# main--/rust-lz-fear

Hardware: AMD Instinct MI355X
Metric: GiB/s compress + decompress, 4 MiB independent blocks, 1/2/4/8 MI355X (higher is better)
Workload: dtype u8

## Files before the change

rust-lz-fear_amd/build.py:

```python
import hashlib
import os
import subprocess
from concurrent.futures import ThreadPoolExecutor

PKG_DIR = os.path.dirname(os.path.abspath(__file__))
CSRC = os.path.join(PKG_DIR, "csrc")
ROOT = os.path.dirname(PKG_DIR)
LIB_PATH = os.environ.get("LZF_LIB_PATH") or os.path.join(PKG_DIR, "liblzfear_hip.so")
ANALYSIS_LIB_PATH = os.path.join(PKG_DIR, "liblzfear_hip_analysis.so")

PRODUCT_HIP = ["capi.hip", "lz4_decompress_batched.hip", "lz4_decompress_paired.hip", "lz4_decompress_seg.hip", "lz4_decompress_fed.hip", "lz4_decoded_size.hip", "lz4_compress.hip",
               "lz4_compress_compact.hip", "lz4_compress_team.hip", "aux_kernels.hip", "frame_device.hip"]
ANALYSIS_HIP = ["analysis/lz4_decompress.hip"]
CXX_SOURCES = ["frame.cpp", "host_staging.cpp"]
HEADERS = ["kernels.h", "lzf_device.h", "lz4_decompress_batch_phase.inc", "lz4_decompress_parse_phase.inc", "lz4_decompress_feed_phase.inc",
           "analysis/capi_analysis.inc",
           "lzf_copy_helpers.h", "lzf_parse_helpers.h", "lzf_compress_common.h", "lzf_simt.h", "lz4_compress_team.inc",
           "host_staging.h", "lzf_frame_scan.h", "lzf_stream_walk.h", "frame_jobs.h", "lzf_frame_layout.h", "lzf_size_rules.h", "lzf_chain_step.h", "frame_deliver_body.inc",
           os.path.join(ROOT, "include", "lzfear_hip.h"), os.path.join(ROOT, "include", "lzfear_frame.h")]


def _path(d):
    return d if os.path.isabs(d) else os.path.join(CSRC, d)


def hipcc():
    for c in ("/opt/rocm/bin/hipcc", "hipcc"):
        if os.path.isabs(c) and os.path.exists(c):
            return c
    return "hipcc"


def _sources(analysis):
# ... 89 lines not shown
```

rust-lz-fear_amd/csrc/capi.hip:

```cpp
#include <hip/hip_runtime.h>
#include <cstdio>
#include <cstdlib>
#include <cstring>
#include <string>
#include <mutex>
#include <vector>
#include "kernels.h"
#include "host_staging.h"

namespace {

thread_local std::string g_last_error;
thread_local const char* g_last_decompress = "";
thread_local const char* g_last_compress = "";

int fail_hip(hipError_t e, const char* what) {
    char buf[256];
    snprintf(buf, sizeof buf, "%s: %s", what, hipGetErrorString(e));
    g_last_error = buf;
    return LZF_E_HIP;
}
#define HIP_TRY(expr)                                          \
    do {                                                       \
        hipError_t e__ = (expr);                               \
// ... 346 lines not shown
    (void)hipGetLastError();
    if (!answer.slots) {
        const uint32_t by_lds = per_cu(kFedLdsAlloc);
        answer.slots = (by_lds < kFedWavesPerCu ? by_lds : kFedWavesPerCu) * cu_count();
    }
#ifdef LZF_ANALYSIS
    if (getenv("LZF_FED_VERBOSE")) fprintf(stderr, "[lzf] bitmap-fed kernel: %u workgroups resident at once (%u compute units), XCD mask 0x%x\n", answer.slots, cu_count(), answer.xcc_mask);
#endif
    by_dev[dev] = answer;
    return answer;
}
struct FedCall {
    SegScratch s; const lzf_decompress_job* jobs = nullptr; lzf_job_result* res = nullptr; uint32_t n = 0; const uint32_t* perm = nullptr;
    size_t o_tick = 0, o_fst = 0; bool live = false;
};
int fed_front(FedCall& f, const lzf_decompress_job* d_jobs, lzf_job_result* d_results, uint32_t n, const uint32_t* perm, hipStream_t st, uint64_t max_in_hint) {
    f.jobs = d_jobs; f.res = d_results; f.n = n; f.perm = perm; f.live = false;
    lzf::seg_ctx& c = f.s.ctx;
    c = lzf::seg_ctx{};
    c.jobs = d_jobs; c.results = d_results; c.n_jobs = n;
    const uint32_t max_in = max_in_hint < kSegMaxIn ? (uint32_t)(max_in_hint < lzf::kSegChunk ? lzf::kSegChunk : max_in_hint) : kSegMaxIn;
    c.max_in = max_in; c.min_in = fed_min_in();
    c.maxch = seg_nch_host(max_in);
    c.maxtile = (max_in + lzf::kSegTile - 1u) / lzf::kSegTile;
    c.n_cu = cu_count();
    c.g_off = 0u; c.g_n = n; c.fed = 1u;
    size_t off = 0;
    auto take = [&](size_t bytes) { const size_t o = off; off = align_up(off + bytes, 256); return o; };
    const size_t o_st = take(sizeof(lzf::seg_job) * (size_t)n);
    const size_t o_top = take(sizeof(unsigned long long));
    const size_t o_x = take(sizeof(uint32_t) * (size_t)n * c.maxch);
    const size_t o_vf = take(sizeof(uint32_t) * (size_t)n * c.maxch);
    const size_t o_bits = take(sizeof(uint32_t) * (size_t)n * c.maxch * lzf::kSegChunkWords);
    f.o_tick = take(sizeof(uint32_t) * 32u * lzf::kFedTicketStride);
    f.o_fst = take(sizeof(lzf::fed_state) * (size_t)n);
    if (off > kFedMaxScratch) return LZF_OK;
    if (hipMallocAsync(&f.s.base, off, st) != hipSuccess) { (void)hipGetLastError(); f.s.base = nullptr; return LZF_OK; }
    uint8_t* b = static_cast<uint8_t*>(f.s.base);
    c.st = reinterpret_cast<lzf::seg_job*>(b + o_st);
    c.rec_top = reinterpret_cast<unsigned long long*>(b + o_top);
    c.xexit = reinterpret_cast<uint32_t*>(b + o_x);
    c.vfrom = reinterpret_cast<uint32_t*>(b + o_vf);
    c.bits = reinterpret_cast<uint32_t*>(b + o_bits);
    f.live = true;
    const int rc = seg_launch(c, 3u, st);
    if (rc != LZF_OK) { (void)hipFreeAsync(f.s.base, st); f.s.base = nullptr; f.live = false; g_last_error = "bitmap-fed decompress: launch failed"; }
    return rc;
}
int fed_back(FedCall& f, hipStream_t st, uint32_t slots_per_cu) {
    if (!f.live) return LZF_OK;
    lzf::seg_ctx& c = f.s.ctx;
    const uint32_t n = f.n;
    uint8_t* b = static_cast<uint8_t*>(f.s.base);
    const FedGeometry fg = fed_geometry(st);
    uint32_t slots = fg.slots;
    if (slots_per_cu && slots_per_cu * cu_count() < slots) slots = slots_per_cu * cu_count();
    uint32_t pieces = n > slots && fg.xcc_mask ? 16u : 1u;
    uint32_t pad = 0;
#ifdef LZF_ANALYSIS
    { static const long e = [] { const char* v = getenv("LZF_FED_PIECES"); return v ? atol(v) : 0L; }(); if (e >= 1 && e <= 4096) pieces = (uint32_t)e; }
    { static const long e = [] { const char* v = getenv("LZF_FED_SLOTS"); return v ? atol(v) : 0L; }(); if (e > 0 && !slots_per_cu) slots = (uint32_t)e * cu_count(); }
    { static const uint32_t e = [] { const char* v = getenv("LZF_FED_PAD_LDS"); return v ? (uint32_t)atol(v) : 0u; }(); pad = e; }
#endif
    if ((uint64_t)n * pieces > 0xFFFFFFF0ull) pieces = 1u;
    if (!fg.xcc_mask) pieces = 1u;
    int rc = LZF_OK;
    lzf::fed_args a{f.jobs, f.res, c.st, c.bits, c.vfrom, f.perm, reinterpret_cast<lzf::fed_state*>(b + f.o_fst), reinterpret_cast<uint32_t*>(b + f.o_tick), fg.xcc_mask ? fg.xcc_mask : 1u, n, c.maxch, pieces, nullptr};
    hipLaunchKernelGGL(lzf::lzf_fed_reset_kernel, dim3((n + 255u) / 256u), dim3(256), 0, st, a);
    hipLaunchKernelGGL(k_fed32, dim3(slots < n ? slots : n), dim3(64), pad, st, a);
    if (hipGetLastError() != hipSuccess) rc = LZF_E_HIP;
    if (rc == LZF_OK) {
        hipLaunchKernelGGL(k_paired24, dim3(n), dim3(128), 0, st, f.jobs, f.res, n, f.perm, (const lzf::seg_job*)c.st);
        if (hipGetLastError() != hipSuccess) rc = LZF_E_HIP;
    }
    if (hipFreeAsync(f.s.base, st) != hipSuccess && rc == LZF_OK) rc = LZF_E_HIP;
    f.s.base = nullptr; f.live = false;
    if (rc != LZF_OK) g_last_error = "bitmap-fed decompress: launch failed";
    return rc;
}
int fed_decompress(const lzf_decompress_job* d_jobs, lzf_job_result* d_results, uint32_t n, const uint32_t* perm, hipStream_t st, bool* used, uint64_t max_in_hint) {
    *used = false;
    if (n > kFedMaxJobs || max_in_hint <= fed_min_in() || max_in_hint <= fed_min_hint()) return LZF_OK;
    FedCall f;
    int rc = fed_front(f, d_jobs, d_results, n, perm, st, max_in_hint);
    if (rc != LZF_OK || !f.live) return rc;
    *used = true;
    return fed_back(f, st, 0u);
}

#ifdef LZF_ANALYSIS
#include "analysis/capi_analysis.inc"
#endif

}

extern "C" {

int lzf_abi_version(void) { return LZFEAR_ABI_VERSION; }
const char* lzf_last_error(void) { return g_last_error.c_str(); }
// ... 84 lines not shown
    if (rc < 0) return rc;
    hipStream_t st = static_cast<hipStream_t>(hip_stream);
    keep_pool_memory();
    uint32_t use_order = 1u;
    bool perm_ok = true;
#ifdef LZF_ANALYSIS
    const int forced = analysis_decompress_variant();
    { static const uint32_t order = analysis_order("LZF_DECOMPRESS_ORDER"); use_order = order; }
    if (forced != kVariantAuto) perm_ok = analysis_perm_ok(forced);
#endif
    AsyncScratch perm_owner; perm_owner.st = st;
    uint32_t* perm = nullptr;
    if (perm_ok && (use_order == 2u || (use_order == 1u && n_jobs > per_cu(20u * 1024u) * cu_count()))) {
        if (hipMallocAsync(&perm_owner.p, 2u * sizeof(uint32_t) * (size_t)n_jobs, st) != hipSuccess) { (void)hipGetLastError(); perm_owner.p = nullptr; }
        perm = static_cast<uint32_t*>(perm_owner.p);
        if (perm) {
            uint32_t* const est = perm + n_jobs;
            uint32_t len_shift = 2u;
#ifdef LZF_ANALYSIS
            { static const uint32_t k = [] { const char* e = getenv("LZF_ORDER_LEN_SHIFT"); return e ? (uint32_t)atol(e) : 2u; }(); len_shift = k; }
#endif
            LAUNCH(lzf::lzf_decompress_cost_kernel, dim3(n_jobs), dim3(64), 0, st, d_jobs, n_jobs, est, len_shift);
            LAUNCH(lzf::lzf_order_by_estimate_kernel, dim3(1), dim3(1024), 0, st, (const uint32_t*)est, perm, n_jobs);
        }
    }
    const uint32_t* cperm = perm;
#ifdef LZF_ANALYSIS
    if (forced != kVariantAuto) {
        g_last_decompress = "analysis variant (LZF_DECOMPRESS_KERNEL)";
        rc = analysis_launch_decompress(forced, d_jobs, d_results, n_jobs, cperm, st);
        HIP_TRY(perm_owner.release());
        return rc;
    }
#endif
    uint32_t seg_min_in = kSegMinIn; bool seg_on = n_jobs <= seg_max_jobs();
#ifdef LZF_ANALYSIS
    { static const int mode = [] { const char* e = getenv("LZF_DECOMPRESS_KERNEL"); return !e ? 0 : !strcmp(e, "seg") ? 1 : (!strcmp(e, "noseg") || !strcmp(e, "fed")) ? 2 : 0; }();
      static const uint32_t min_in = [] { const char* e = getenv("LZF_SEG_MIN_IN"); return e ? (uint32_t)atol(e) : 0u; }();
      if (mode == 1) { seg_on = true; seg_min_in = min_in; }
      if (mode == 2) seg_on = false; }
#endif
    if (seg_on) {
        bool used = false; uint32_t ring = 0;
        rc = seg_decompress(d_jobs, d_results, n_jobs, seg_min_in, st, &used, max_input_len, &ring);
        if (used) g_last_decompress = ring == 131072u ? "segmented: lzf_seg_resolve_pair_kernel<131072> + lzf_decompress_paired_kernel<4096,48,640>"
                                     : ring == 65536u ? "segmented: lzf_seg_resolve_pair_kernel<65536> + lzf_decompress_paired_kernel<4096,48,640>"
                                                      : "segmented: lzf_seg_resolve_pair_kernel<32768> + lzf_decompress_paired_kernel<4096,48,640>";
        if (rc != LZF_OK || used) { HIP_TRY(perm_owner.release()); return rc; }
    }
    const uint32_t resident48 = per_cu(20u * 1024u) * cu_count();
    const uint32_t resident24 = per_cu(12800u) * cu_count();
    bool fed_on = n_jobs > resident24;
#ifdef LZF_ANALYSIS
    { static const int mode = [] { const char* e = getenv("LZF_DECOMPRESS_KERNEL"); return !e ? 0 : !strcmp(e, "fed") ? 1 : !strcmp(e, "nofed") ? 2 : 0; }();
      if (mode == 1) fed_on = true;
      if (mode == 2) fed_on = false; }
#endif
    if (fed_on) {
        bool used = false;
        rc = fed_decompress(d_jobs, d_results, n_jobs, cperm, st, &used, max_input_len);
        if (used) g_last_decompress = "bitmap-fed: lzf_seg_parse_kernel + lzf_decompress_fed_kernel<4096,32,352> + lzf_decompress_paired_kernel<4096,24,384>";
        if (rc != LZF_OK || used) { HIP_TRY(perm_owner.release()); return rc; }
    }
    g_last_decompress = n_jobs <= resident48 ? "lzf_decompress_paired_kernel<4096,48,640>" : n_jobs <= 8u * resident48 ? "lzf_decompress_paired_kernel<4096,24,384>"
                                                                                                             : "lzf_decompress_batched_kernel<4096,16,256,staged>";
    if (n_jobs <= resident48)
        LAUNCH(k_paired48, dim3(n_jobs), dim3(128), 0, st, d_jobs, d_results, n_jobs, cperm, (const lzf::seg_job*)nullptr);
    else if (n_jobs <= 8u * resident48)
        LAUNCH(k_paired24, dim3(n_jobs), dim3(128), 0, st, d_jobs, d_results, n_jobs, cperm, (const lzf::seg_job*)nullptr);
    else
        LAUNCH(k_staged16, dim3(n_jobs), dim3(64), 0, st, d_jobs, d_results, n_jobs, cperm);
    HIP_TRY(perm_owner.release());
    return LZF_OK;
}

int lzf_decompressed_size_batch(const lzf_decompress_job* d_jobs, lzf_job_result* d_results, uint32_t n_jobs, uint64_t max_input_len, void* hip_stream) {
    (void)max_input_len;
    if (n_jobs == 0) return LZF_OK;
// ... 410 lines not shown
```

rust-lz-fear_amd/csrc/kernels.h:

```cpp
#pragma once
#include "lzf_device.h"

namespace lzf {
#ifdef LZF_ANALYSIS
__global__ void lzf_decompress_wave_kernel(const lzf_decompress_job* __restrict__ jobs,
                                           lzf_job_result* __restrict__ results, uint32_t n_jobs, const uint32_t* __restrict__ perm);
#endif
template <int RING, int S, int TOKCAP, bool STAGE>
__global__ __launch_bounds__(64) void lzf_decompress_batched_kernel(const lzf_decompress_job* __restrict__ jobs,
                                              lzf_job_result* __restrict__ results, uint32_t n_jobs, const uint32_t* __restrict__ perm);
#ifdef LZF_ANALYSIS
#define LZF_DECOMPRESS_VARIANTS(X) \
    X(staged16, 4096, 16, 256, true)    \
    X(staged32, 4096, 32, 512, true)    \
    X(direct4w, 4096, 256, 2048, false)
#else
#define LZF_DECOMPRESS_VARIANTS(X) X(staged16, 4096, 16, 256, true)
#endif
#define LZF_EXT(NAME, R, S_, T, ST) extern template __global__ void lzf_decompress_batched_kernel<R, S_, T, ST>(const lzf_decompress_job*, lzf_job_result*, uint32_t, const uint32_t*);
LZF_DECOMPRESS_VARIANTS(LZF_EXT)
#undef LZF_EXT
template <int S, int TOKCAP>
__global__ __launch_bounds__(64) void lzf_decoded_size_kernel(const lzf_decompress_job* __restrict__ jobs, lzf_job_result* __restrict__ results,
                                                              uint32_t n_jobs, uint32_t* __restrict__ ticket, const uint32_t* __restrict__ perm);
// ... 33 lines not shown
    uint32_t* tile_tok;
    uint32_t* tile_out;
    u32x4* recs;
    unsigned long long* rec_top;
    uint64_t rec_cap;
    uint32_t n_jobs, maxch, maxtile, max_in, min_in;
    uint32_t ring_bytes;
    uint32_t* order;
    uint32_t n_cu;
    uint32_t* by_len;
    uint32_t rec_by_len;
    uint32_t dbg_force;
    uint32_t g_off, g_n, grouped;
    uint32_t res_prio;
    uint32_t fed;
};
struct fed_state { uint32_t flag, cstart, expect, o; };
constexpr uint32_t kFedEnded = 0x80000000u;
constexpr uint32_t kFedTicketStride = 32u;
struct fed_args {
    const lzf_decompress_job* jobs;
    lzf_job_result* results;
    seg_job* st;
    const uint32_t* bits;
    const uint32_t* vfrom;
    const uint32_t* perm;
    fed_state* state;
    uint32_t* ticket;
    uint32_t xcc_mask;
    uint32_t n_jobs, maxch;
    uint32_t pieces;
    uint32_t* census;
};
__global__ void lzf_fed_reset_kernel(fed_args a);
#define LZF_FED_VARIANTS(X) X(fed32, 4096, 32, 352)
#ifdef LZF_DBG_FED_WAVES
#define LZF_FED_WAVES LZF_DBG_FED_WAVES
#else
#define LZF_FED_WAVES 6
#endif
#if LZF_FED_WAVES > 0
#define LZF_FED_BOUNDS __launch_bounds__(64, LZF_FED_WAVES)
#else
#define LZF_FED_BOUNDS __launch_bounds__(64)
#endif
template <int RING, int W, int TOKCAP>
__global__ LZF_FED_BOUNDS void lzf_decompress_fed_kernel(fed_args a);
#define LZF_EXTF(NAME, RG, W_, T) extern template __global__ void lzf_decompress_fed_kernel<RG, W_, T>(fed_args);
LZF_FED_VARIANTS(LZF_EXTF)
#undef LZF_EXTF
__device__ __forceinline__ uint32_t seg_job_of(const seg_ctx& c, uint32_t i) { return c.by_len ? c.by_len[i + c.g_off] : i + c.g_off; }
constexpr uint32_t kSegRegion = 256, kSegChunk = 64u * kSegRegion, kSegOverlap = 2048, kSegStride = kSegChunk - kSegOverlap;
constexpr uint32_t kSegChunkWords = kSegChunk / 32u, kSegTile = 2048;
__global__ void lzf_seg_plan_kernel(seg_ctx c);
__global__ void lzf_seg_order_kernel(seg_ctx c);
__global__ void lzf_seg_pause_kernel(uint32_t ticks);
__global__ void lzf_seg_rank_kernel(seg_ctx c, uint32_t* __restrict__ by_tok, uint4 group_sizes);
__global__ void lzf_seg_by_len_kernel(seg_ctx c);
__global__ void lzf_seg_parse_kernel(seg_ctx c);
__global__ void lzf_seg_seam_kernel(seg_ctx c);
__global__ void lzf_seg_tilesum_kernel(seg_ctx c);
__global__ void lzf_seg_scan_kernel(seg_ctx c);
__global__ void lzf_seg_records_kernel(seg_ctx c);
template <int R>
__global__ __launch_bounds__(128) void lzf_seg_resolve_pair_kernel(seg_ctx c);
extern template __global__ void lzf_seg_resolve_pair_kernel<32768>(seg_ctx);
extern template __global__ void lzf_seg_resolve_pair_kernel<65536>(seg_ctx);
extern template __global__ void lzf_seg_resolve_pair_kernel<131072>(seg_ctx);
// ... 36 lines not shown
```

rust-lz-fear_amd/csrc/lz4_decompress_batch_phase.inc:

```
            uint32_t tidx = 0;
            if (LZF_DBG_SKIP & 1) { tidx = Tc; o += Tc; }
            while (tidx < Tc && status == LZF_OK) {
                PHASE(0);
#if defined(LZF_DBG_ROUNDS) && defined(LZF_DBG_ROUNDS_HERE)
                ++dbg_batches;
#endif
                const uint32_t ob0 = o;
                const uint32_t nb_try = Tc - tidx < kWave ? Tc - tidx : kWave;
                const bool act0 = lane < nb_try;
                uint32_t L = 0, M = 0, src = 0;
                bool has = false;
#if defined(LZF_FED_DECODE)
                uint32_t next;
                const uint32_t pos = toks[act0 ? tidx + lane : tidx];
                const uint32_t tp = cstart + pos;
                uint32_t w;
                asm volatile("ds_read_b32 %0, %1\n\ts_waitcnt lgkmcnt(0)" : "=v"(w) : "v"(cbuf_a + pos) : "memory");
                const uint32_t l0 = (w >> 4) & 15u, b1 = (w >> 8) & 255u, m0 = w & 15u;
                const bool lx = l0 == 15u;
                L = l0 + (lx ? b1 : 0u);
                src = tp + (lx ? 2u : 1u);
                const uint32_t q = src + L;
                has = q + 2u <= len;
                const bool mx = has && m0 == 15u;
// ... 329 lines not shown
```

rust-lz-fear_amd/csrc/lz4_decompress_fed.hip:

```cpp
#include "lzf_device.h"
#include "kernels.h"
#include "lzf_copy_helpers.h"

namespace lzf {

__device__ __forceinline__ uint32_t xcc_id() {
    uint32_t v; asm volatile("s_getreg_b32 %0, hwreg(HW_REG_XCC_ID)" : "=s"(v)); return v & 15u;
}

template <int RING, int W, int TOKCAP>
__global__ LZF_FED_BOUNDS void lzf_decompress_fed_kernel(fed_args a) {
    constexpr bool STAGE = true;
    constexpr uint32_t kMask = RING - 1;
    constexpr uint32_t kSpanMax = RING / 3;
    constexpr uint32_t kNearHist = RING - kSpanMax;
    constexpr uint32_t kRound = 32u * (uint32_t)W;
    constexpr uint32_t kCB = kRound + 128u;
    static_assert(W >= 1 && W <= 64 && (kSegTile % kRound) == 0, "a round is one bit-map word per lane and subdivides a tile");
    static_assert(TOKCAP >= (int)(kRound / 3u + 1u), "a round's tokens (at least three bytes each) fit the list");
    static_assert(kCB % 16 == 0, "the round is staged in 16-byte pieces");
    __shared__ __attribute__((aligned(16))) uint8_t ring[RING];
    __shared__ __attribute__((aligned(16))) uint8_t cbuf[kCB];
    __shared__ __attribute__((aligned(16))) uint16_t toks[TOKCAP];

    const uint32_t lane = threadIdx.x;
    if (a.census) {
        if (lane == 0u) {
            __hip_atomic_fetch_or(&a.census[2], 1u << (xcc_id() & 31u), __ATOMIC_RELAXED, __HIP_MEMORY_SCOPE_AGENT);
            __hip_atomic_fetch_add(&a.census[0], 1u, __ATOMIC_RELAXED, __HIP_MEMORY_SCOPE_AGENT);
            const unsigned long long t0 = wall_clock64();
            while (wall_clock64() - t0 < 30000ull) __builtin_amdgcn_s_sleep(16);
            const uint32_t seen = __hip_atomic_load(&a.census[0], __ATOMIC_RELAXED, __HIP_MEMORY_SCOPE_AGENT);
            __hip_atomic_fetch_min(&a.census[1], seen, __ATOMIC_RELAXED, __HIP_MEMORY_SCOPE_AGENT);
// ... 16 lines not shown
    const seg_job sj = a.st[jid];
    if (!sj.eligible || sj.failed || sj.done) continue;
    LZF_GLOBAL fed_state* const fs = (LZF_GLOBAL fed_state*)a.state + jid;
    const lzf_decompress_job job = a.jobs[jid];
    const long long t_start = clock64();
#ifdef LZF_DBG_TIMELINE
    const unsigned long long t_wall0 = wall_clock64();
#endif

    int status = LZF_OK;
    bool bailed = false, parked = false;
    uint32_t o = 0;
#ifdef LZF_DBG_PHASE_SEL
    long long ph_acc_out = 0;
#endif
    if (job.input_len >= kMaxPosB || job.out_existing_len >= kMaxPosB || job.prefix_len >= kMaxPosB || job.out_existing_len > job.out_cap) continue;
    {
        cgu8* __restrict__ in = as_global(job.input);
        cgu8* __restrict__ prefix = as_global(job.prefix);
        gu8* out = as_global(job.out);
        const uint32_t len = (uint32_t)job.input_len;
        const uint32_t plen = (uint32_t)job.prefix_len;
        const uint32_t cap = job.out_cap > kMaxPosB ? kMaxPosB : (uint32_t)job.out_cap;
        const uint64_t limit = job.output_limit;
        const uint32_t rb = (uint32_t)(reinterpret_cast<uintptr_t>(out) & 15u);
        const uint32_t ring_a = lds_addr(ring), cbuf_a = lds_addr(cbuf);
        const LZF_GLOBAL uint32_t* const fed_bits = (const LZF_GLOBAL uint32_t*)a.bits + (size_t)jid * a.maxch * kSegChunkWords;
        const LZF_GLOBAL uint32_t* const fed_vf = (const LZF_GLOBAL uint32_t*)a.vfrom + (size_t)jid * a.maxch;
#define RIDX(x) (((x) + rb) & kMask)

        auto ring_fill = [&](uint32_t a_, uint32_t b) {
            uint32_t nh = (16u - ((a_ + rb) & 15u)) & 15u; if (nh > b - a_) nh = b - a_;
            if (lane < nh) ring[RIDX(a_ + lane)] = out[a_ + lane];
            a_ += nh;
            const uint32_t nchunks = (b - a_) >> 4;
            for (uint32_t c = lane; c < nchunks; c += kWave)
                *reinterpret_cast<u32x4*>(&ring[RIDX(a_ + 16u * c)]) = *reinterpret_cast<const LZF_GLOBAL u32x4*>(out + a_ + 16u * c);
            a_ += nchunks << 4;
            if (lane < b - a_) ring[RIDX(a_ + lane)] = out[a_ + lane];
        };
        auto ring_flush = [&](uint32_t a_, uint32_t b) {
            uint32_t nh = (16u - ((a_ + rb) & 15u)) & 15u; if (nh > b - a_) nh = b - a_;
            if (lane < nh) out[a_ + lane] = ring[RIDX(a_ + lane)];
// ... 8 lines not shown
        uint32_t expect = 0;
        uint32_t cstart = 0;
        o = (uint32_t)job.out_existing_len;
        const uint32_t rounds = (len + kRound - 1u) / kRound, per = (rounds + pieces - 1u) / pieces;
        const uint32_t piece_end = (piece + 1u) * per >= rounds ? len : (piece + 1u) * per * kRound;
        if (piece > 0u) {
            uint32_t f = 0;
            for (uint32_t spin = 0; spin < (1u << 22); ++spin) {
                f = __hip_atomic_load(&fs->flag, __ATOMIC_RELAXED, __HIP_MEMORY_SCOPE_AGENT);
                if (f >= piece) break;
                __builtin_amdgcn_s_sleep(32);
            }
            f = __builtin_amdgcn_readfirstlane(f);
            if (f != piece) continue;
            __builtin_amdgcn_fence(__ATOMIC_ACQUIRE, "agent");
            cstart = fs->cstart; expect = fs->expect; o = fs->o;
        }
        uint32_t safe = o;
        if (o > 0) ring_fill(o > (uint32_t)RING ? o - RING : 0u, o);
#ifdef LZF_DBG_PHASE_SEL
        long long ph_t = clock64(), ph_acc = 0;
#define PHASE(i) do { const long long tn__ = clock64(); if ((i) == LZF_DBG_PHASE_SEL) ph_acc += tn__ - ph_t; ph_t = tn__; } while (0)
#else
#define PHASE(i) do { } while (0)
#endif
        while (cstart < len && expect < len && status == LZF_OK) {
            if (cstart >= piece_end) { parked = true; break; }
            __syncthreads();
#include "lz4_decompress_feed_phase.inc"
            if (Tc) {
#define LZF_FED_DECODE
#ifdef LZF_FED_FAR_LATE
#define LZF_FAR_LATE
#endif
#include "lz4_decompress_batch_phase.inc"
#undef LZF_FAR_LATE
#undef LZF_FED_DECODE
            }
            if (bail) { bailed = true; break; }
            const uint32_t nx = expect & ~(kRound - 1u);
            cstart = nx > cstart ? nx : cstart + kRound;
        }
        if (!parked && status == LZF_OK && expect < len) bailed = true;
#ifdef LZF_DBG_PHASE_SEL
        ph_acc_out = ph_acc;
#endif
#undef PHASE
#undef RIDX
        if (parked && status == LZF_OK && !bailed) {
            if (lane == 0u) { fs->cstart = cstart; fs->expect = expect; fs->o = o; }
            __builtin_amdgcn_fence(__ATOMIC_RELEASE, "workgroup");
            asm volatile("s_waitcnt vmcnt(0)" ::: "memory");
            if (lane == 0u) __hip_atomic_store(&fs->flag, piece + 1u, __ATOMIC_RELAXED, __HIP_MEMORY_SCOPE_AGENT);
            continue;
        }
    }
    if (pieces > 1u && lane == 0u) __hip_atomic_store(&fs->flag, kFedEnded, __ATOMIC_RELAXED, __HIP_MEMORY_SCOPE_AGENT);
    if (bailed || status != LZF_OK) continue;
    if (lane == 0) {
        a.results[jid].out_len = o;
        a.results[jid].status = LZF_OK;
#ifdef LZF_DBG_PHASE_SEL
        a.results[jid].reserved = (uint32_t)(ph_acc_out >> 10);
#elif defined(LZF_DBG_TIMELINE)
        a.results[jid].reserved = (uint32_t)(((t_wall0 >> 8) & 0xFFFFull) << 16) | (uint32_t)((wall_clock64() >> 8) & 0xFFFFull);
#else
        a.results[jid].reserved = (uint32_t)((clock64() - t_start) >> 10);
#endif
        a.st[jid].done = 1u;
    }
    }
}

__global__ __launch_bounds__(256) void lzf_fed_reset_kernel(fed_args a) {
    const uint32_t k = blockIdx.x * blockDim.x + threadIdx.x;
    if (k < 32u) a.ticket[k * kFedTicketStride] = 0u;
    if (k < a.n_jobs) a.state[k].flag = 0u;
// ... 8 lines not shown
```

rust-lz-fear_amd/csrc/lz4_decompress_feed_phase.inc:

```
            uint32_t Tc = 0;
            bool bail = false;
            auto rdb = [&](uint32_t q) -> uint32_t {
                const uint32_t r = q - cstart;
                if (r < kCB) return lds_ld8(cbuf_a + r);
                return (uint32_t)in[q];
            };
            if (expect < cstart + kRound) {
                {
                    const uint32_t avail = len - cstart < kCB ? len - cstart : kCB;
                    cgu8* g = in + cstart;
                    constexpr uint32_t kPieces = (kCB + 1023u) / 1024u;
                    u32x4 v[kPieces];
#pragma unroll
                    for (uint32_t k = 0; k < kPieces; ++k) {
                        const uint32_t i = k * 1024u + lane * 16u;
                        v[k] = u32x4{0, 0, 0, 0};
                        if (i + 16u <= avail) v[k] = ld16(g + i);
                        else if (i < avail) { for (uint32_t t = 0; i + t < avail; ++t) v[k][(t >> 2) & 3u] |= (uint32_t)g[i + t] << ((t & 3u) * 8u); }
                    }
                    const uint32_t h = cstart < kSegChunk ? 0u : 1u + (cstart - kSegChunk) / kSegStride;
                    uint32_t w = 0;
                    if (lane < (uint32_t)W) {
                        w = fed_bits[(size_t)h * kSegChunkWords + ((cstart - h * kSegStride) >> 5) + lane];
                        const uint32_t vf = fed_vf[h];
                        const uint32_t wpos = cstart + lane * 32u;
                        if (vf == 0xFFFFFFFFu || vf >= wpos + 32u) w = 0u;
                        else if (vf > wpos) w &= ~((1u << (vf - wpos)) - 1u);
                        if (wpos >= len) w = 0u;
                        else if (len - wpos < 32u) w &= (1u << (len - wpos)) - 1u;
                    }
#pragma unroll
                    for (uint32_t k = 0; k < kPieces; ++k) {
                        const uint32_t i = k * 1024u + lane * 16u;
                        if (i < kCB) *reinterpret_cast<u32x4*>(&cbuf[i]) = v[k];
                    }
                    PHASE(6);
                    const uint32_t cnt = (uint32_t)__popc(w);
                    const uint32_t incl = wave_scan_add(cnt);
                    uint32_t k = incl - cnt;
                    Tc = __builtin_amdgcn_readlane(incl, 63);
                    if (Tc > (uint32_t)TOKCAP) { bail = true; Tc = 0; }
                    else while (w) { const uint32_t b = (uint32_t)__builtin_ctz(w); toks[k++] = lane * 32u + b; w &= w - 1u; }
                }
                PHASE(7);
                if (Tc == 0u && !bail) bail = true;
                if (bail) Tc = 0;
            }
```

rust-lz-fear_amd/csrc/lz4_decompress_seg.hip:

```cpp
#include "lzf_device.h"
#include "kernels.h"
#include "lzf_copy_helpers.h"
#include <type_traits>

namespace lzf {
namespace {

constexpr uint32_t S = kSegRegion;
constexpr uint32_t kCB = kSegChunk;
constexpr uint32_t kNone = 0xFFFFFFFFu;
constexpr uint32_t kLenClamp = 1u << 26;
constexpr uint32_t kTileStage = kSegTile + 128u;
constexpr uint32_t kTileTokMax = kSegTile / 3u + 2u;
constexpr uint32_t kFlagCoop = 1u;

struct __attribute__((packed, aligned(1))) S8B { uint64_t v; };
struct __attribute__((packed, aligned(1))) S4B { uint32_t v; };
struct __attribute__((packed, aligned(1))) S2B { uint16_t v; };
__device__ __forceinline__ void st8(gu8* p, uint64_t v) { reinterpret_cast<LZF_GLOBAL S8B*>(p)->v = v; }
__device__ __forceinline__ void st4(gu8* p, uint32_t v) { reinterpret_cast<LZF_GLOBAL S4B*>(p)->v = v; }
__device__ __forceinline__ void st2(gu8* p, uint32_t v) { reinterpret_cast<LZF_GLOBAL S2B*>(p)->v = (uint16_t)v; }

__device__ __forceinline__ void copy_small_gg(gu8* d, cgu8* g, uint32_t n) {
    if (n > 32u) {
// ... 87 lines not shown

__global__ __launch_bounds__(256) void lzf_seg_plan_kernel(seg_ctx c) {
    const uint32_t j = blockIdx.x * blockDim.x + threadIdx.x;
    if (j == 0u) *c.rec_top = 0ull;
    if (j >= c.n_jobs) return;
    const lzf_decompress_job job = c.jobs[j];
    seg_job s;
    s.failed = 0; s.done = 0; s.ntok = 0; s.outb = 0; s.pad = 0; s.rec_off = 0; s.pad2 = 0;
    s.eligible = ((c.fed || (job.prefix_len == 0 && job.out_existing_len == 0)) && job.input_len >= c.min_in && job.input_len <= c.max_in &&
                  job.input != nullptr && job.out != nullptr) ? 1u : 0u;
    const uint32_t len = s.eligible ? (uint32_t)job.input_len : 0u;
    s.nch = s.eligible ? seg_nch(len) : 0u;
    s.ntile = (len + kSegTile - 1u) / kSegTile;
    if (s.nch > c.maxch || s.ntile > c.maxtile) { s.eligible = 0; s.nch = 0; s.ntile = 0; }
    c.st[j] = s;
}

__global__ __launch_bounds__(64) void lzf_seg_parse_kernel(seg_ctx c) {
    __shared__ __attribute__((aligned(16))) uint8_t lds_parse[2u * 64u * 8u * 4u + kCB];
    static_assert(sizeof(lds_parse) == 20480, "eight chunks per CU: an eighth of 160 KiB each");
    uint32_t* const rowsA = reinterpret_cast<uint32_t*>(lds_parse);
    uint32_t* const rowsB = rowsA + 64u * 8u;
    const uint32_t j = seg_job_of(c, blockIdx.y);
    const seg_job sj = c.st[j];
    if (!sj.eligible) return;
    const uint32_t lane = threadIdx.x & 63u;
    const lzf_decompress_job job = c.jobs[j];
    cgu8* __restrict__ in = as_global(job.input);
    const uint32_t len = (uint32_t)job.input_len;
    uint8_t* const cbuf = lds_parse + 2u * 64u * 8u * 4u;
// ... 200 lines not shown
                else { X = x1; mpos = end_r; }
            }
        }
        {
            const uint32_t mb = mpos - rb0;
            u32x4 o0, o1;
#pragma unroll
            for (uint32_t i = 0; i < 8u; ++i) {
                const uint32_t wb = mb >> 5;
                const uint32_t keep = i < wb ? 0u : i == wb ? ~((1u << (mb & 31u)) - 1u) : ~0u;
                const uint32_t v = in_input ? ((ROWA(i) & keep) | ROWB(i)) : 0u;
                if (i < 4u) o0[i] = v; else o1[i - 4u] = v;
            }
            LZF_GLOBAL u32x4* dst = (LZF_GLOBAL u32x4*)(c.bits + ((size_t)j * c.maxch + h) * kSegChunkWords + lane * 8u);
            dst[0] = o0; dst[1] = o1;
            const uint32_t xm = __builtin_amdgcn_readlane(wave_scan_max(X), 63);
            uint64_t xe = (uint64_t)cstart + xm;
            if (xe > len) xe = len;
            if (lane == 0u) c.xexit[(size_t)j * c.maxch + h] = (uint32_t)xe;
        }
    }
}

#undef ROWA
#undef ROWB

__global__ __launch_bounds__(64) void lzf_seg_seam_kernel(seg_ctx c) {
    __shared__ uint16_t patch[kSegStride / 3u + 8u];
    constexpr uint32_t kWin = 2048;
    __shared__ __attribute__((aligned(16))) uint8_t wbytes[kWin + 128u];
    __shared__ uint32_t wbits[kWin / 32u + 2u];
    if (blockIdx.x >= c.g_n) return;
    const uint32_t j = c.grouped ? seg_job_of(c, blockIdx.x) : blockIdx.x;
    const seg_job sj = c.st[j];
// ... 1082 lines not shown
```

rust-lz-fear_amd/csrc/lzf_device.h:

```cpp
#pragma once
#if !defined(LZF_ANALYSIS) && (defined(LZF_DBG_SKIP) || defined(LZF_DBG_SKIP2) || defined(LZF_DBG_TIME) || defined(LZF_DBG_COUNT) || defined(LZF_DBG_DRY_MAIN) || defined(LZF_DBG_LDS_PAD) || defined(LZF_DBG_PATHS) || defined(LZF_DBG_PHASE_SEL) || defined(LZF_DBG_ROUNDS) || defined(LZF_DBG_TIMELINE) || defined(LZF_DBG_NOFENCE) || \
    defined(LZF_SEG_DBG_SKIP) || defined(LZF_SEG_DBG_NOWAIT) || defined(LZF_SEG_TIME) || defined(LZF_SEG_NOASM) || defined(LZF_SEG_NORLE))
#error "LZF_DBG_* / LZF_SEG_* instrumentation is for -DLZF_ANALYSIS builds only"
#endif
#include <hip/hip_runtime.h>
#include <stdint.h>
#include "../../include/lzfear_hip.h"

namespace lzf {

constexpr uint32_t kWave = 64;

typedef uint32_t u32x4 __attribute__((ext_vector_type(4)));
typedef uint32_t u32x2 __attribute__((ext_vector_type(2)));
struct __attribute__((packed, aligned(1))) U16B { u32x4 v; };
struct __attribute__((packed, aligned(1))) U8B { uint64_t v; };
struct __attribute__((packed, aligned(1))) U4B { uint32_t v; };
struct __attribute__((packed, aligned(1))) U2B { uint16_t v; };

#define LZF_GLOBAL __attribute__((address_space(1)))
typedef LZF_GLOBAL uint8_t gu8;
typedef const LZF_GLOBAL uint8_t cgu8;
template <typename T> __device__ __forceinline__ cgu8* as_global(const T* p) { return (cgu8*)p; }
template <typename T> __device__ __forceinline__ gu8* as_global(T* p) { return (gu8*)p; }
// ... 76 lines not shown
```

Baseline: 489.2.

## Slide fed decode windows from expect and fold ordering estimate into seg plan

Measured after the change: 514.2, median of 6. 1.05x the previous value.

```diff
diff --git a/rust-lz-fear_amd/build.py b/rust-lz-fear_amd/build.py
--- a/rust-lz-fear_amd/build.py
+++ b/rust-lz-fear_amd/build.py
@@ -16,7 +16,7 @@
 HEADERS = ["kernels.h", "lzf_device.h", "lz4_decompress_batch_phase.inc", "lz4_decompress_parse_phase.inc", "lz4_decompress_feed_phase.inc",
            "analysis/capi_analysis.inc",
            "lzf_copy_helpers.h", "lzf_parse_helpers.h", "lzf_compress_common.h", "lzf_simt.h", "lz4_compress_team.inc",
-           "host_staging.h", "lzf_frame_scan.h", "lzf_stream_walk.h", "frame_jobs.h", "lzf_frame_layout.h", "lzf_size_rules.h", "lzf_chain_step.h", "frame_deliver_body.inc",
+           "host_staging.h", "lzf_frame_scan.h", "lzf_stream_walk.h", "frame_jobs.h", "lzf_frame_layout.h", "lzf_size_rules.h", "lzf_chain_step.h", "lzf_fed_window.h", "frame_deliver_body.inc",
            os.path.join(ROOT, "include", "lzfear_hip.h"), os.path.join(ROOT, "include", "lzfear_frame.h")]
 
 
diff --git a/rust-lz-fear_amd/csrc/capi.hip b/rust-lz-fear_amd/csrc/capi.hip
--- a/rust-lz-fear_amd/csrc/capi.hip
+++ b/rust-lz-fear_amd/csrc/capi.hip
@@ -384,7 +384,7 @@
     SegScratch s; const lzf_decompress_job* jobs = nullptr; lzf_job_result* res = nullptr; uint32_t n = 0; const uint32_t* perm = nullptr;
     size_t o_tick = 0, o_fst = 0; bool live = false;
 };
-int fed_front(FedCall& f, const lzf_decompress_job* d_jobs, lzf_job_result* d_results, uint32_t n, const uint32_t* perm, hipStream_t st, uint64_t max_in_hint) {
+int fed_front(FedCall& f, const lzf_decompress_job* d_jobs, lzf_job_result* d_results, uint32_t n, uint32_t* perm, uint32_t* est, uint32_t len_shift, hipStream_t st, uint64_t max_in_hint) {
     f.jobs = d_jobs; f.res = d_results; f.n = n; f.perm = perm; f.live = false;
     lzf::seg_ctx& c = f.s.ctx;
     c = lzf::seg_ctx{};
@@ -395,12 +395,11 @@
     c.maxtile = (max_in + lzf::kSegTile - 1u) / lzf::kSegTile;
     c.n_cu = cu_count();
     c.g_off = 0u; c.g_n = n; c.fed = 1u;
+    c.est = perm ? est : nullptr; c.len_shift = len_shift;
     size_t off = 0;
     auto take = [&](size_t bytes) { const size_t o = off; off = align_up(off + bytes, 256); return o; };
     const size_t o_st = take(sizeof(lzf::seg_job) * (size_t)n);
     const size_t o_top = take(sizeof(unsigned long long));
-    const size_t o_x = take(sizeof(uint32_t) * (size_t)n * c.maxch);
-    const size_t o_vf = take(sizeof(uint32_t) * (size_t)n * c.maxch);
     const size_t o_bits = take(sizeof(uint32_t) * (size_t)n * c.maxch * lzf::kSegChunkWords);
     f.o_tick = take(sizeof(uint32_t) * 32u * lzf::kFedTicketStride);
     f.o_fst = take(sizeof(lzf::fed_state) * (size_t)n);
@@ -409,11 +408,13 @@
     uint8_t* b = static_cast<uint8_t*>(f.s.base);
     c.st = reinterpret_cast<lzf::seg_job*>(b + o_st);
     c.rec_top = reinterpret_cast<unsigned long long*>(b + o_top);
-    c.xexit = reinterpret_cast<uint32_t*>(b + o_x);
-    c.vfrom = reinterpret_cast<uint32_t*>(b + o_vf);
     c.bits = reinterpret_cast<uint32_t*>(b + o_bits);
     f.live = true;
-    const int rc = seg_launch(c, 3u, st);
+    int rc = seg_launch(c, 2u, st);
+    if (rc == LZF_OK && c.est) {
+        hipLaunchKernelGGL(lzf::lzf_order_by_estimate_kernel, dim3(1), dim3(1024), 0, st, (const uint32_t*)est, perm, n);
+        if (hipGetLastError() != hipSuccess) rc = LZF_E_HIP;
+    }
     if (rc != LZF_OK) { (void)hipFreeAsync(f.s.base, st); f.s.base = nullptr; f.live = false; g_last_error = "bitmap-fed decompress: launch failed"; }
     return rc;
 }
@@ -435,7 +436,11 @@
     if ((uint64_t)n * pieces > 0xFFFFFFF0ull) pieces = 1u;
     if (!fg.xcc_mask) pieces = 1u;
     int rc = LZF_OK;
-    lzf::fed_args a{f.jobs, f.res, c.st, c.bits, c.vfrom, f.perm, reinterpret_cast<lzf::fed_state*>(b + f.o_fst), reinterpret_cast<uint32_t*>(b + f.o_tick), fg.xcc_mask ? fg.xcc_mask : 1u, n, c.maxch, pieces, nullptr};
+    uint32_t carry = (uint32_t)kFedwCarry;
+#ifdef LZF_ANALYSIS
+    { static const long e = [] { const char* v = getenv("LZF_FED_CARRY"); return v ? atol(v) : -1L; }(); if (e >= 0 && e < 64) carry = (uint32_t)e; }
+#endif
+    lzf::fed_args a{f.jobs, f.res, c.st, c.bits, f.perm, reinterpret_cast<lzf::fed_state*>(b + f.o_fst), reinterpret_cast<uint32_t*>(b + f.o_tick), fg.xcc_mask ? fg.xcc_mask : 1u, n, c.maxch, pieces, carry, nullptr};
     hipLaunchKernelGGL(lzf::lzf_fed_reset_kernel, dim3((n + 255u) / 256u), dim3(256), 0, st, a);
     hipLaunchKernelGGL(k_fed32, dim3(slots < n ? slots : n), dim3(64), pad, st, a);
     if (hipGetLastError() != hipSuccess) rc = LZF_E_HIP;
@@ -448,11 +453,11 @@
     if (rc != LZF_OK) g_last_error = "bitmap-fed decompress: launch failed";
     return rc;
 }
-int fed_decompress(const lzf_decompress_job* d_jobs, lzf_job_result* d_results, uint32_t n, const uint32_t* perm, hipStream_t st, bool* used, uint64_t max_in_hint) {
+int fed_decompress(const lzf_decompress_job* d_jobs, lzf_job_result* d_results, uint32_t n, uint32_t* perm, uint32_t* est, uint32_t len_shift, hipStream_t st, bool* used, uint64_t max_in_hint) {
     *used = false;
     if (n > kFedMaxJobs || max_in_hint <= fed_min_in() || max_in_hint <= fed_min_hint()) return LZF_OK;
     FedCall f;
-    int rc = fed_front(f, d_jobs, d_results, n, perm, st, max_in_hint);
+    int rc = fed_front(f, d_jobs, d_results, n, perm, est, len_shift, st, max_in_hint);
     if (rc != LZF_OK || !f.live) return rc;
     *used = true;
     return fed_back(f, st, 0u);
@@ -567,19 +572,24 @@
     if (perm_ok && (use_order == 2u || (use_order == 1u && n_jobs > per_cu(20u * 1024u) * cu_count()))) {
         if (hipMallocAsync(&perm_owner.p, 2u * sizeof(uint32_t) * (size_t)n_jobs, st) != hipSuccess) { (void)hipGetLastError(); perm_owner.p = nullptr; }
         perm = static_cast<uint32_t*>(perm_owner.p);
-        if (perm) {
-            uint32_t* const est = perm + n_jobs;
-            uint32_t len_shift = 2u;
-#ifdef LZF_ANALYSIS
-            { static const uint32_t k = [] { const char* e = getenv("LZF_ORDER_LEN_SHIFT"); return e ? (uint32_t)atol(e) : 2u; }(); len_shift = k; }
-#endif
-            LAUNCH(lzf::lzf_decompress_cost_kernel, dim3(n_jobs), dim3(64), 0, st, d_jobs, n_jobs, est, len_shift);
-            LAUNCH(lzf::lzf_order_by_estimate_kernel, dim3(1), dim3(1024), 0, st, (const uint32_t*)est, perm, n_jobs);
-        }
-    }
+    }
+    uint32_t* const est = perm ? perm + n_jobs : nullptr;
+    uint32_t len_shift = 2u;
+#ifdef LZF_ANALYSIS
+    { static const uint32_t k = [] { const char* e = getenv("LZF_ORDER_LEN_SHIFT"); return e ? (uint32_t)atol(e) : 2u; }(); len_shift = k; }
+#endif
+    bool ordered = false;
+    auto order_by_sampling = [&]() -> int {
+        if (!perm || ordered) return LZF_OK;
+        ordered = true;
+        LAUNCH(lzf::lzf_decompress_cost_kernel, dim3(n_jobs), dim3(64), 0, st, d_jobs, n_jobs, est, len_shift);
+        LAUNCH(lzf::lzf_order_by_estimate_kernel, dim3(1), dim3(1024), 0, st, (const uint32_t*)est, perm, n_jobs);
+        return LZF_OK;
+    };
     const uint32_t* cperm = perm;
 #ifdef LZF_ANALYSIS
     if (forced != kVariantAuto) {
+        if ((rc = order_by_sampling()) != LZF_OK) { HIP_TRY(perm_owner.release()); return rc; }
         g_last_decompress = "analysis variant (LZF_DECOMPRESS_KERNEL)";
         rc = analysis_launch_decompress(forced, d_jobs, d_results, n_jobs, cperm, st);
         HIP_TRY(perm_owner.release());
@@ -594,6 +604,7 @@
       if (mode == 2) seg_on = false; }
 #endif
     if (seg_on) {
+        if ((rc = order_by_sampling()) != LZF_OK) { HIP_TRY(perm_owner.release()); return rc; }
         bool used = false; uint32_t ring = 0;
         rc = seg_decompress(d_jobs, d_results, n_jobs, seg_min_in, st, &used, max_input_len, &ring);
         if (used) g_last_decompress = ring == 131072u ? "segmented: lzf_seg_resolve_pair_kernel<131072> + lzf_decompress_paired_kernel<4096,48,640>"
@@ -611,10 +622,11 @@
 #endif
     if (fed_on) {
         bool used = false;
-        rc = fed_decompress(d_jobs, d_results, n_jobs, cperm, st, &used, max_input_len);
+        rc = fed_decompress(d_jobs, d_results, n_jobs, perm, est, len_shift, st, &used, max_input_len);
         if (used) g_last_decompress = "bitmap-fed: lzf_seg_parse_kernel + lzf_decompress_fed_kernel<4096,32,352> + lzf_decompress_paired_kernel<4096,24,384>";
         if (rc != LZF_OK || used) { HIP_TRY(perm_owner.release()); return rc; }
     }
+    if ((rc = order_by_sampling()) != LZF_OK) { HIP_TRY(perm_owner.release()); return rc; }
     g_last_decompress = n_jobs <= resident48 ? "lzf_decompress_paired_kernel<4096,48,640>" : n_jobs <= 8u * resident48 ? "lzf_decompress_paired_kernel<4096,24,384>"
                                                                                                              : "lzf_decompress_batched_kernel<4096,16,256,staged>";
     if (n_jobs <= resident48)
diff --git a/rust-lz-fear_amd/csrc/kernels.h b/rust-lz-fear_amd/csrc/kernels.h
--- a/rust-lz-fear_amd/csrc/kernels.h
+++ b/rust-lz-fear_amd/csrc/kernels.h
@@ -1,5 +1,6 @@
 #pragma once
 #include "lzf_device.h"
+#include "lzf_fed_window.h"
 
 namespace lzf {
 #ifdef LZF_ANALYSIS
@@ -71,8 +72,10 @@
     uint32_t g_off, g_n, grouped;
     uint32_t res_prio;
     uint32_t fed;
+    uint32_t* est;
+    uint32_t len_shift;
 };
-struct fed_state { uint32_t flag, cstart, expect, o; };
+struct fed_state { uint32_t flag, expect, o, pad; };
 constexpr uint32_t kFedEnded = 0x80000000u;
 constexpr uint32_t kFedTicketStride = 32u;
 struct fed_args {
@@ -80,13 +83,13 @@
     lzf_job_result* results;
     seg_job* st;
     const uint32_t* bits;
-    const uint32_t* vfrom;
     const uint32_t* perm;
     fed_state* state;
     uint32_t* ticket;
     uint32_t xcc_mask;
     uint32_t n_jobs, maxch;
     uint32_t pieces;
+    uint32_t carry;
     uint32_t* census;
 };
 __global__ void lzf_fed_reset_kernel(fed_args a);
@@ -109,6 +112,7 @@
 __device__ __forceinline__ uint32_t seg_job_of(const seg_ctx& c, uint32_t i) { return c.by_len ? c.by_len[i + c.g_off] : i + c.g_off; }
 constexpr uint32_t kSegRegion = 256, kSegChunk = 64u * kSegRegion, kSegOverlap = 2048, kSegStride = kSegChunk - kSegOverlap;
 constexpr uint32_t kSegChunkWords = kSegChunk / 32u, kSegTile = 2048;
+static_assert(kSegChunk == (uint32_t)kFedwChunk && kSegOverlap == (uint32_t)kFedwOverlap && kSegStride == (uint32_t)kFedwStride, "lzf_fed_window.h restates the chunk geometry");
 __global__ void lzf_seg_plan_kernel(seg_ctx c);
 __global__ void lzf_seg_order_kernel(seg_ctx c);
 __global__ void lzf_seg_pause_kernel(uint32_t ticks);
diff --git a/rust-lz-fear_amd/csrc/lz4_decompress_batch_phase.inc b/rust-lz-fear_amd/csrc/lz4_decompress_batch_phase.inc
--- a/rust-lz-fear_amd/csrc/lz4_decompress_batch_phase.inc
+++ b/rust-lz-fear_amd/csrc/lz4_decompress_batch_phase.inc
@@ -1,9 +1,18 @@
             uint32_t tidx = 0;
             if (LZF_DBG_SKIP & 1) { tidx = Tc; o += Tc; }
+#if defined(LZF_FED_DECODE)
+            if (LZF_DBG_SKIP & 1) expect = len;
+#endif
             while (tidx < Tc && status == LZF_OK) {
+#if defined(LZF_FED_DECODE)
+                if (lzf_fedw_carry(Tc, tidx, cstart + kRound, len, fed_carry)) break;
+#endif
                 PHASE(0);
 #if defined(LZF_DBG_ROUNDS) && defined(LZF_DBG_ROUNDS_HERE)
                 ++dbg_batches;
+#endif
+#if defined(LZF_FED_DECODE) && defined(LZF_DBG_FED_COUNT)
+                ++dbg_fed[0];
 #endif
                 const uint32_t ob0 = o;
                 const uint32_t nb_try = Tc - tidx < kWave ? Tc - tidx : kWave;
diff --git a/rust-lz-fear_amd/csrc/lz4_decompress_fed.hip b/rust-lz-fear_amd/csrc/lz4_decompress_fed.hip
--- a/rust-lz-fear_amd/csrc/lz4_decompress_fed.hip
+++ b/rust-lz-fear_amd/csrc/lz4_decompress_fed.hip
@@ -1,6 +1,7 @@
 #include "lzf_device.h"
 #include "kernels.h"
 #include "lzf_copy_helpers.h"
+#include "lzf_fed_window.h"
 
 namespace lzf {
 
@@ -16,7 +17,7 @@
     constexpr uint32_t kNearHist = RING - kSpanMax;
     constexpr uint32_t kRound = 32u * (uint32_t)W;
     constexpr uint32_t kCB = kRound + 128u;
-    static_assert(W >= 1 && W <= 64 && (kSegTile % kRound) == 0, "a round is one bit-map word per lane and subdivides a tile");
+    static_assert(W >= 1 && W <= 64 && kRound == (uint32_t)kFedwRound, "a window is one bit-map word per lane (whose owner is worked out per word: lzf_fed_window.h)");
     static_assert(TOKCAP >= (int)(kRound / 3u + 1u), "a round's tokens (at least three bytes each) fit the list");
     static_assert(kCB % 16 == 0, "the round is staged in 16-byte pieces");
     __shared__ __attribute__((aligned(16))) uint8_t ring[RING];
@@ -63,6 +64,9 @@
 #ifdef LZF_DBG_PHASE_SEL
     long long ph_acc_out = 0;
 #endif
+#ifdef LZF_DBG_FED_COUNT
+    uint32_t dbg_fed[3] = {0u, 0u, 0u};
+#endif
     if (job.input_len >= kMaxPosB || job.out_existing_len >= kMaxPosB || job.prefix_len >= kMaxPosB || job.out_existing_len > job.out_cap) continue;
     {
         cgu8* __restrict__ in = as_global(job.input);
@@ -75,7 +79,6 @@
         const uint32_t rb = (uint32_t)(reinterpret_cast<uintptr_t>(out) & 15u);
         const uint32_t ring_a = lds_addr(ring), cbuf_a = lds_addr(cbuf);
         const LZF_GLOBAL uint32_t* const fed_bits = (const LZF_GLOBAL uint32_t*)a.bits + (size_t)jid * a.maxch * kSegChunkWords;
-        const LZF_GLOBAL uint32_t* const fed_vf = (const LZF_GLOBAL uint32_t*)a.vfrom + (size_t)jid * a.maxch;
 #define RIDX(x) (((x) + rb) & kMask)
 
         auto ring_fill = [&](uint32_t a_, uint32_t b) {
@@ -114,7 +117,7 @@
             f = __builtin_amdgcn_readfirstlane(f);
             if (f != piece) continue;
             __builtin_amdgcn_fence(__ATOMIC_ACQUIRE, "agent");
-            cstart = fs->cstart; expect = fs->expect; o = fs->o;
+            expect = fs->expect; o = fs->o;
         }
         uint32_t safe = o;
         if (o > 0) ring_fill(o > (uint32_t)RING ? o - RING : 0u, o);
@@ -124,9 +127,25 @@
 #else
 #define PHASE(i) do { } while (0)
 #endif
-        while (cstart < len && expect < len && status == LZF_OK) {
-            if (cstart >= piece_end) { parked = true; break; }
+#if defined(LZF_FED_FIXED_ROUNDS)
+        constexpr int kFixed = 1;
+        const uint32_t fed_carry = 0u;
+#elif defined(LZF_ANALYSIS)
+        constexpr int kFixed = 0;
+        const uint32_t fed_carry = a.carry < kWave ? a.carry : kWave - 1u;
+#else
+        constexpr int kFixed = 0;
+        constexpr uint32_t fed_carry = kFedwCarry;
+#endif
+        bool fed_walk = false;
+        while (expect < len && status == LZF_OK) {
+            if (expect >= piece_end) { parked = true; break; }
+            const uint32_t expect_in = expect;
+            cstart = lzf_fedw_start(expect, kFixed);
             __syncthreads();
+#ifdef LZF_DBG_FED_COUNT
+            ++dbg_fed[fed_walk ? 2 : 1];
+#endif
 #include "lz4_decompress_feed_phase.inc"
             if (Tc) {
 #define LZF_FED_DECODE
@@ -137,18 +156,20 @@
 #undef LZF_FAR_LATE
 #undef LZF_FED_DECODE
             }
-            if (bail) { bailed = true; break; }
-            const uint32_t nx = expect & ~(kRound - 1u);
-            cstart = nx > cstart ? nx : cstart + kRound;
-        }
-        if (!parked && status == LZF_OK && expect < len) bailed = true;
+            if (bail) {
+                if (fed_walk) { bailed = true; break; }
+                fed_walk = true; continue;
+            }
+            fed_walk = false;
+            if (expect == expect_in && status == LZF_OK) { bailed = true; break; }
+        }
 #ifdef LZF_DBG_PHASE_SEL
         ph_acc_out = ph_acc;
 #endif
 #undef PHASE
 #undef RIDX
         if (parked && status == LZF_OK && !bailed) {
-            if (lane == 0u) { fs->cstart = cstart; fs->expect = expect; fs->o = o; }
+            if (lane == 0u) { fs->expect = expect; fs->o = o; }
             __builtin_amdgcn_fence(__ATOMIC_RELEASE, "workgroup");
             asm volatile("s_waitcnt vmcnt(0)" ::: "memory");
             if (lane == 0u) __hip_atomic_store(&fs->flag, piece + 1u, __ATOMIC_RELAXED, __HIP_MEMORY_SCOPE_AGENT);
@@ -160,7 +181,9 @@
     if (lane == 0) {
         a.results[jid].out_len = o;
         a.results[jid].status = LZF_OK;
-#ifdef LZF_DBG_PHASE_SEL
+#ifdef LZF_DBG_FED_COUNT
+        a.results[jid].reserved = dbg_fed[LZF_DBG_FED_COUNT];
+#elif defined(LZF_DBG_PHASE_SEL)
         a.results[jid].reserved = (uint32_t)(ph_acc_out >> 10);
 #elif defined(LZF_DBG_TIMELINE)
         a.results[jid].reserved = (uint32_t)(((t_wall0 >> 8) & 0xFFFFull) << 16) | (uint32_t)((wall_clock64() >> 8) & 0xFFFFull);
diff --git a/rust-lz-fear_amd/csrc/lz4_decompress_feed_phase.inc b/rust-lz-fear_amd/csrc/lz4_decompress_feed_phase.inc
--- a/rust-lz-fear_amd/csrc/lz4_decompress_feed_phase.inc
+++ b/rust-lz-fear_amd/csrc/lz4_decompress_feed_phase.inc
@@ -5,7 +5,7 @@
                 if (r < kCB) return lds_ld8(cbuf_a + r);
                 return (uint32_t)in[q];
             };
-            if (expect < cstart + kRound) {
+            {
                 {
                     const uint32_t avail = len - cstart < kCB ? len - cstart : kCB;
                     cgu8* g = in + cstart;
@@ -18,16 +18,14 @@
                         if (i + 16u <= avail) v[k] = ld16(g + i);
                         else if (i < avail) { for (uint32_t t = 0; i + t < avail; ++t) v[k][(t >> 2) & 3u] |= (uint32_t)g[i + t] << ((t & 3u) * 8u); }
                     }
-                    const uint32_t h = cstart < kSegChunk ? 0u : 1u + (cstart - kSegChunk) / kSegStride;
                     uint32_t w = 0;
-                    if (lane < (uint32_t)W) {
-                        w = fed_bits[(size_t)h * kSegChunkWords + ((cstart - h * kSegStride) >> 5) + lane];
-                        const uint32_t vf = fed_vf[h];
-                        const uint32_t wpos = cstart + lane * 32u;
-                        if (vf == 0xFFFFFFFFu || vf >= wpos + 32u) w = 0u;
-                        else if (vf > wpos) w &= ~((1u << (vf - wpos)) - 1u);
-                        if (wpos >= len) w = 0u;
-                        else if (len - wpos < 32u) w &= (1u << (len - wpos)) - 1u;
+                    const uint32_t wpos = cstart + lane * 32u;
+                    if (!fed_walk && lane < (uint32_t)W && wpos < len) {
+                        const uint32_t h = lzf_fedw_chunk(wpos);
+                        w = fed_bits[(size_t)h * kSegChunkWords + lzf_fedw_word(wpos, h)];
+                        if (expect >= wpos + 32u) w = 0u;
+                        else if (expect > wpos) w &= ~((1u << (expect - wpos)) - 1u);
+                        if (len - wpos < 32u) w &= (1u << (len - wpos)) - 1u;
                     }
 #pragma unroll
                     for (uint32_t k = 0; k < kPieces; ++k) {
@@ -35,14 +33,35 @@
                         if (i < kCB) *reinterpret_cast<u32x4*>(&cbuf[i]) = v[k];
                     }
                     PHASE(6);
-                    const uint32_t cnt = (uint32_t)__popc(w);
-                    const uint32_t incl = wave_scan_add(cnt);
-                    uint32_t k = incl - cnt;
-                    Tc = __builtin_amdgcn_readlane(incl, 63);
-                    if (Tc > (uint32_t)TOKCAP) { bail = true; Tc = 0; }
-                    else while (w) { const uint32_t b = (uint32_t)__builtin_ctz(w); toks[k++] = lane * 32u + b; w &= w - 1u; }
+                    if (!fed_walk) {
+                        const uint32_t cnt = (uint32_t)__popc(w);
+                        const uint32_t incl = wave_scan_add(cnt);
+                        uint32_t k = incl - cnt;
+                        Tc = __builtin_amdgcn_readlane(incl, 63);
+                        if (Tc > (uint32_t)TOKCAP) { bail = true; Tc = 0; }
+                        else while (w) { const uint32_t b = (uint32_t)__builtin_ctz(w); toks[k++] = lane * 32u + b; w &= w - 1u; }
+                        if (Tc == 0u) bail = true;
+                    } else {
+                        uint32_t np = 0, werr = 0;
+                        if (lane == 0u) {
+                            uint32_t p = expect;
+                            while (p - cstart < kRound && p < len && np < (uint32_t)TOKCAP) {
+                                toks[np++] = (uint16_t)(p - cstart);
+                                const uint32_t tok = rdb(p);
+                                uint32_t q = p + 1u, L = tok >> 4, b = 0;
+                                if (L == 15u) { do { if (q >= len) { werr = 1u; break; } b = rdb(q); ++q; L += b; if (L > kMaxPosB) L = kMaxPosB; } while (b == 255u); }
+                                if (werr || len - q < L) { werr = 1u; break; }
+                                q += L;
+                                if (len - q < 2u) { p = len; break; }
+                                q += 2u;
+                                if ((tok & 15u) == 15u) { do { if (q >= len) { werr = 1u; break; } b = rdb(q); ++q; } while (b == 255u); }
+                                if (werr) break;
+                                p = q;
+                            }
+                        }
+                        Tc = __builtin_amdgcn_readfirstlane(np);
+                        if (__builtin_amdgcn_readfirstlane(werr) || Tc == 0u) { bail = true; Tc = 0; }
+                    }
                 }
                 PHASE(7);
-                if (Tc == 0u && !bail) bail = true;
-                if (bail) Tc = 0;
             }
diff --git a/rust-lz-fear_amd/csrc/lz4_decompress_seg.hip b/rust-lz-fear_amd/csrc/lz4_decompress_seg.hip
--- a/rust-lz-fear_amd/csrc/lz4_decompress_seg.hip
+++ b/rust-lz-fear_amd/csrc/lz4_decompress_seg.hip
@@ -125,6 +125,10 @@
     s.ntile = (len + kSegTile - 1u) / kSegTile;
     if (s.nch > c.maxch || s.ntile > c.maxtile) { s.eligible = 0; s.nch = 0; s.ntile = 0; }
     c.st[j] = s;
+    if (c.est) {
+        const uint32_t l31 = job.input_len > 0x7FFFFFFFull ? 0x7FFFFFFFu : (uint32_t)job.input_len;
+        c.est[j] = (s.eligible ? 0u : l31 >> 4) + (c.len_shift < 32u ? l31 >> c.len_shift : 0u);
+    }
 }
 
 __global__ __launch_bounds__(64) void lzf_seg_parse_kernel(seg_ctx c) {
@@ -355,10 +359,18 @@
             }
             LZF_GLOBAL u32x4* dst = (LZF_GLOBAL u32x4*)(c.bits + ((size_t)j * c.maxch + h) * kSegChunkWords + lane * 8u);
             dst[0] = o0; dst[1] = o1;
-            const uint32_t xm = __builtin_amdgcn_readlane(wave_scan_max(X), 63);
-            uint64_t xe = (uint64_t)cstart + xm;
-            if (xe > len) xe = len;
-            if (lane == 0u) c.xexit[(size_t)j * c.maxch + h] = (uint32_t)xe;
+            if (!c.fed) {
+                const uint32_t xm = __builtin_amdgcn_readlane(wave_scan_max(X), 63);
+                uint64_t xe = (uint64_t)cstart + xm;
+                if (xe > len) xe = len;
+                if (lane == 0u) c.xexit[(size_t)j * c.maxch + h] = (uint32_t)xe;
+            }
+            if (c.est) {
+                uint32_t cnt = 0;
+                if (h == 0u || rb0 >= kSegOverlap) cnt = (uint32_t)(__popc(o0[0]) + __popc(o0[1]) + __popc(o0[2]) + __popc(o0[3]) + __popc(o1[0]) + __popc(o1[1]) + __popc(o1[2]) + __popc(o1[3]));
+                const uint32_t tot = __builtin_amdgcn_readlane(wave_scan_add(cnt), 63);
+                if (lane == 0u) __hip_atomic_fetch_add(&c.est[j], tot, __ATOMIC_RELAXED, __HIP_MEMORY_SCOPE_AGENT);
+            }
         }
     }
 }
diff --git a/rust-lz-fear_amd/csrc/lzf_device.h b/rust-lz-fear_amd/csrc/lzf_device.h
--- a/rust-lz-fear_amd/csrc/lzf_device.h
+++ b/rust-lz-fear_amd/csrc/lzf_device.h
@@ -1,5 +1,5 @@
 #pragma once
-#if !defined(LZF_ANALYSIS) && (defined(LZF_DBG_SKIP) || defined(LZF_DBG_SKIP2) || defined(LZF_DBG_TIME) || defined(LZF_DBG_COUNT) || defined(LZF_DBG_DRY_MAIN) || defined(LZF_DBG_LDS_PAD) || defined(LZF_DBG_PATHS) || defined(LZF_DBG_PHASE_SEL) || defined(LZF_DBG_ROUNDS) || defined(LZF_DBG_TIMELINE) || defined(LZF_DBG_NOFENCE) || \
+#if !defined(LZF_ANALYSIS) && (defined(LZF_DBG_SKIP) || defined(LZF_DBG_SKIP2) || defined(LZF_DBG_TIME) || defined(LZF_DBG_COUNT) || defined(LZF_DBG_DRY_MAIN) || defined(LZF_DBG_LDS_PAD) || defined(LZF_DBG_PATHS) || defined(LZF_DBG_PHASE_SEL) || defined(LZF_DBG_ROUNDS) || defined(LZF_DBG_FED_COUNT) || defined(LZF_DBG_TIMELINE) || defined(LZF_DBG_NOFENCE) || \
     defined(LZF_SEG_DBG_SKIP) || defined(LZF_SEG_DBG_NOWAIT) || defined(LZF_SEG_TIME) || defined(LZF_SEG_NOASM) || defined(LZF_SEG_NORLE))
 #error "LZF_DBG_* / LZF_SEG_* instrumentation is for -DLZF_ANALYSIS builds only"
 #endif
diff --git a/rust-lz-fear_amd/csrc/lzf_fed_window.h b/rust-lz-fear_amd/csrc/lzf_fed_window.h
--- /dev/null
+++ b/rust-lz-fear_amd/csrc/lzf_fed_window.h
@@ -0,0 +1,37 @@
+#ifndef LZF_FED_WINDOW_H
+#define LZF_FED_WINDOW_H
+
+#include <stdint.h>
+
+#if defined(__HIPCC__) || defined(__CUDACC__)
+#define LZF_FEDW_HD __host__ __device__ static inline
+#else
+#define LZF_FEDW_HD static inline
+#endif
+
+enum {
+    kFedwChunk = 16384,
+    kFedwOverlap = 2048,
+    kFedwStride = kFedwChunk - kFedwOverlap,
+    kFedwRound = 1024,
+    kFedwLanes = 64,
+    kFedwCarry = 32
+};
+#if defined(__cplusplus)
+static_assert(kFedwChunk % 32 == 0 && kFedwOverlap % 32 == 0 && kFedwStride % 32 == 0, "a 32-aligned bit-map word has one owner");
+#endif
+
+LZF_FEDW_HD uint32_t lzf_fedw_start(uint32_t expect, int fixed) {
+    return fixed ? expect & ~(uint32_t)(kFedwRound - 1) : expect & ~31u;
+}
+LZF_FEDW_HD uint32_t lzf_fedw_chunk(uint32_t wpos) {
+    return wpos < (uint32_t)kFedwChunk ? 0u : 1u + (wpos - (uint32_t)kFedwChunk) / (uint32_t)kFedwStride;
+}
+LZF_FEDW_HD uint32_t lzf_fedw_word(uint32_t wpos, uint32_t h) {
+    return (wpos - h * (uint32_t)kFedwStride) >> 5;
+}
+LZF_FEDW_HD int lzf_fedw_carry(uint32_t tc, uint32_t tidx, uint32_t window_end, uint32_t len, uint32_t carry) {
+    return tidx > 0u && tc - tidx <= carry && window_end < len;
+}
+
+#endif
```
